# WoodOxen/tactics2d

Hardware: NVIDIA H100
Metric: participant_steps_per_sec (higher is better)
Workload: dtype f32

## Files before the change

tactics2d_b200/csrc/t2d_kernels.cu:

```cuda
#include <cuda_runtime.h>
#include <stdint.h>
#include <stdio.h>
#include <string.h>

#include <algorithm>
#include <atomic>
#include <cmath>
#include <memory>
#include <mutex>
#include <string>
#include <vector>

#include "../../include/t2d_b200.h"
#include "t2d_math.cuh"

namespace t2d {

constexpr int MAX_WARPS_PER_CTA = 8;
constexpr int CTA_THREADS = MAX_WARPS_PER_CTA * 32;
constexpr int PPL = 4;
constexpr int POSE_PER_WARP = 32 * PPL;
constexpr int MAP_SMEM_LIMIT = 120 * 1024;

struct MapHeader {
  int32_t n_seg, gx, gy, n_items;
  float x0, y0, inv_cell, cell;
  uint32_t off_seg, off_cell, off_items, total_bytes;
  uint32_t off_clear;
  int32_t fine;
  uint32_t off_dcell, off_ditems;
  float dil;
  int32_t n_ditems;
  uint32_t off_objfirst;
  int32_t n_poly;
  uint32_t off_poly;
  uint32_t off_pbox;
  uint32_t off_fine;
  uint32_t smem_bytes;
  float bxmin, bxmax, bymin, bymax;
  int32_t has_bounds;
  uint32_t pad[3];
};
constexpr float CLEAR_QUANT = 0.125f;
static_assert(sizeof(MapHeader) == 128, "MapHeader must be 128 bytes");

struct StepArgs {
  float *x, *y, *h, *v, *vx, *vy;
  const uint8_t* type_id;
  int32_t* step_count;
  const float* action;
  const float* ego_action;
  uint8_t* flags;
  int16_t* hit_index;
  int16_t* hit_segment;
  uint8_t* scn_status;
  uint8_t* done;
  const unsigned char* map_blob;
  const uint32_t* tile_off;
  const uint16_t* tile_id;
  MapHeader mh;
  const Params* table;
  int map_bytes, map_in_smem;
  int n_types;
  int N, M, G;
  int g_shift, mp_shift, unused1, n_tiles, wpc, table_bytes;
  int off_poseA, off_poseB, off_hit, off_queue, off_sorted, unused0, off_qcount, off_bar;
  int n_steps;
  float dt, dt_rem;
  double dt_d, dt_rem_d, interval_d;
  int max_step, cfg_flags;
  int do_physics, has_bounds, vec_ok, needs_vel_in;
  int prefetch;
  float bxmin, bxmax, bymin, bymax;
  float rb_max;
  const float* goal_target;
  float* goal_iou;
  float* goal_last_pose;
  int32_t* goal_noact_count;
  float goal_threshold;
  int goal_noact_max;
  float *wheel_f, *wheel_r;
};

__device__ __forceinline__ uint32_t smem_u32(const void* p) { return (uint32_t)__cvta_generic_to_shared(p); }

__device__ __forceinline__ void mbar_init(uint64_t* bar, uint32_t count) {
  asm volatile("mbarrier.init.shared::cta.b64 [%0], %1;" ::"r"(smem_u32(bar)), "r"(count));
}
__device__ __forceinline__ void fence_mbar_init() { asm volatile("fence.mbarrier_init.release.cluster;" ::: "memory"); }
__device__ __forceinline__ void mbar_expect_tx(uint64_t* bar, uint32_t bytes) {
  asm volatile("mbarrier.arrive.expect_tx.shared::cta.b64 _, [%0], %1;" ::"r"(smem_u32(bar)), "r"(bytes) : "memory");
}
__device__ __forceinline__ void bulk_g2s(void* dst, const void* src, uint32_t bytes, uint64_t* bar) {
  asm volatile("cp.async.bulk.shared::cluster.global.mbarrier::complete_tx::bytes [%0], [%1], %2, [%3];" ::"r"(
                   smem_u32(dst)),
               "l"(src), "r"(bytes), "r"(smem_u32(bar))
               : "memory");
}
__device__ __forceinline__ void mbar_wait(uint64_t* bar, uint32_t parity) {
  uint32_t ok = 0;
  while (!ok) {
    asm volatile(
        "{\n\t.reg .pred p;\n\t"
        "mbarrier.try_wait.parity.shared::cta.b64 p, [%1], %2;\n\t"
        "selp.u32 %0, 1, 0, p;\n\t}"
        : "=r"(ok)
        : "r"(smem_u32(bar)), "r"(parity)
        : "memory");
  }
}

template <int BYTES> struct VecOf;
template <> struct VecOf<1> { using T = uint8_t; };
template <> struct VecOf<2> { using T = uint16_t; };
template <> struct VecOf<4> { using T = uint32_t; };
template <> struct VecOf<8> { using T = uint2; };
template <> struct VecOf<16> { using T = uint4; };

template <typename T, int N>
__device__ __forceinline__ void ld_vec(const T* p, T (&o)[N]) {
  using V = typename VecOf<sizeof(T) * N>::T;
  const V v = *reinterpret_cast<const V*>(p);
  memcpy(o, &v, sizeof(V));
}
template <typename T, int N>
__device__ __forceinline__ void st_vec(T* p, const T (&o)[N]) {
  using V = typename VecOf<sizeof(T) * N>::T;
  V v;
  memcpy(&v, o, sizeof(V));
  *reinterpret_cast<V*>(p) = v;
}

struct Pose {
  float x, y, h, c, s, l, w;
};

__device__ __noinline__ bool pair_exact(const Pose a, const Pose b) {
  const bool ca = a.w < 0.0f, cb = b.w < 0.0f;
  if (!ca && !cb) return obb_obb_f64(a.x, a.y, a.h, a.l, a.w, b.x, b.y, b.h, b.l, b.w);
  if (!ca && cb) return obb_circle_f64(a.x, a.y, a.h, a.l, a.w, b.x, b.y, b.l);
  if (ca && !cb) return obb_circle_f64(b.x, b.y, b.h, b.l, b.w, a.x, a.y, a.l);
  return circle_circle_f64(a.x, a.y, a.l, b.x, b.y, b.l);
}

__device__ __forceinline__ bool pair_hit(const Pose& a, const Pose& b) {
  const bool ca = a.w < 0.0f, cb = b.w < 0.0f;
  int r;
  if (!ca && !cb) r = obb_obb_f32(a.x, a.y, a.c, a.s, a.l, a.w, b.x, b.y, b.c, b.s, b.l, b.w);
  else if (!ca && cb) r = obb_circle_f32(a.x, a.y, a.c, a.s, a.l, a.w, b.x, b.y, b.l);
  else if (ca && !cb) r = obb_circle_f32(b.x, b.y, b.c, b.s, b.l, b.w, a.x, a.y, a.l);
  else r = circle_circle_f32(a.x, a.y, a.l, b.x, b.y, b.l);
  if (r < 0) return pair_exact(a, b);
  return r != 0;
}

__device__ __noinline__ bool seg_exact(const Pose a, const float4 sg) {
  if (a.w < 0.0f) return circle_segment_f64(a.x, a.y, a.l, sg.x, sg.y, sg.z, sg.w);
  return obb_segment_f64(a.x, a.y, a.h, a.l, a.w, sg.x, sg.y, sg.z, sg.w);
}

__device__ __forceinline__ bool seg_hit(const Pose& a, const float4 sg) {
  int r = a.w < 0.0f ? circle_segment_f32(a.x, a.y, a.l, sg.x, sg.y, sg.z, sg.w)
                     : obb_segment_f32(a.x, a.y, a.c, a.s, a.l, a.w, sg.x, sg.y, sg.z, sg.w);
  if (r < 0) return seg_exact(a, sg);
  return r != 0;
}

__device__ __noinline__ bool oob_exact(const Pose a, float xmin, float xmax, float ymin, float ymax) {
  return out_of_bound_f64(a.x, a.y, a.h, a.l, a.w, a.w < 0.0f, xmin, xmax, ymin, ymax);
}

__device__ __noinline__ void other_model_step(OneIO& io, const Params& p, int n_steps, double dt, double dt_rem, double interval) {
  if (p.model() == MODEL_DYNAMICS) {
    dynamics_step(io, p, n_steps, dt);
  } else if (p.model() == MODEL_POINTMASS_NEWTON) {
    pointmass_newton_step(io, p, interval);
  } else if (p.model() == MODEL_POINTMASS_EULER) {
    pointmass_euler_step(io, p, n_steps, dt, dt_rem);
  } else {
    sincos_fast(io.h, &io.sh, &io.ch);
  }
}

__device__ __forceinline__ unsigned near_fetch(const float ax, const float ay, const float rbound, const MapHeader& mh, const uint8_t* fine,
                                               unsigned& alt) {
  const float r = rbound * 1.0001f + 1e-3f;
  const float fx = (ax - mh.x0) * mh.inv_cell, fy = (ay - mh.y0) * mh.inv_cell;
  const float gxf = (float)mh.gx, gyf = (float)mh.gy;
  const bool inside = fx >= 0.0f && fy >= 0.0f && fx < gxf && fy < gyf;
  const float kf = (float)mh.fine;
  const int nx = mh.gx * mh.fine, ny = mh.gy * mh.fine;
  const float ux = fmaf(inside ? fx : 0.0f, kf, -0.5f), uy = fmaf(inside ? fy : 0.0f, kf, -0.5f);
  int ix = __float_as_int(ux + RINT_MAGIC) - 0x4B400000, iy = __float_as_int(uy + RINT_MAGIC) - 0x4B400000;
  ix = min(max(ix, 0), nx - 1); iy = min(max(iy, 0), ny - 1);
  const unsigned q = (unsigned)__ldg(fine + (size_t)iy * nx + ix);
  const float ox = fmaxf(fmaxf(-fx, fx - gxf), 0.0f), oy = fmaxf(fmaxf(-fy, fy - gyf), 0.0f);
  const unsigned q_out = fmaxf(ox, oy) * mh.cell <= r ? 0u : 255u;
  alt = inside ? 0xffffffffu : q_out;
  return q;
}
__device__ __forceinline__ bool near_decide(unsigned q, unsigned alt, const float rbound) {
  const unsigned v = alt == 0xffffffffu ? q : alt;
  return (float)v * CLEAR_QUANT <= rbound * 1.0001f + 1e-3f;
}

static_assert(PPL == 4, "pslot's masks and shifts are those of 4 participants per lane");
__device__ __forceinline__ int pslot(int slot) { return ((slot & 3) << 5) | (slot >> 2); }

__device__ __forceinline__ Pose load_pose(const float4* poseA, const float4* poseB, int slot) {
  const int idx = pslot(slot);
  const float4 a = poseA[idx], b = poseB[idx];
  Pose p;
  p.x = a.x; p.y = a.y; p.h = a.w; p.c = b.x; p.s = b.y; p.l = b.z; p.w = b.w;
  return p;
}

constexpr int QCAP = 192;

__device__ __forceinline__ void pair_resolve(int ti, int tj, int mp_shift, const float4* poseA, const float4* poseB, int* hitmin) {
  const Pose a = load_pose(poseA, poseB, ti), b = load_pose(poseA, poseB, tj);
  if (pair_hit(a, b)) {
    const int mask = (1 << mp_shift) - 1;
    atomicMin(&hitmin[pslot(ti)], tj & mask);
    atomicMin(&hitmin[pslot(tj)], ti & mask);
  }
}

__device__ __forceinline__ float neg_reach2(float rb, float rb_max) {
  const float rr = rb + rb_max;
  return -fmaf(rr * rr, 1.00001f, 1e-12f);
}

__device__ __forceinline__ unsigned f2ord(float f) {
  const unsigned u = __float_as_uint(f);
  return (u & 0x80000000u) ? ~u : (u | 0x80000000u);
}
__device__ __forceinline__ float ord2f(unsigned o) { return __uint_as_float((o & 0x80000000u) ? (o & 0x7fffffffu) : ~o); }

__device__ __forceinline__ void sweep_pair(const float4& a, const float4& b, int tb, int M, int Mh, unsigned* queue, int* qcount) {
  const int sa = (int)(__float_as_uint(a.w) & 127u), sb = (int)(__float_as_uint(b.w) & 127u);
  int d = sb - sa;
  if (d < 0) d += M;
  const float dx = b.x - a.x, dy = b.y - a.y;
  if (d <= Mh && fmaf(dx, dx, fmaf(dy, dy, a.z)) <= 0.0f) {
    const int slot = atomicAdd(qcount, 1);
    if (slot < QCAP) queue[slot] = ((unsigned)(tb + sa) << 16) | (unsigned)(tb + sb);
  }
  if (d >= M - Mh && fmaf(dx, dx, fmaf(dy, dy, b.z)) <= 0.0f) {
    const int slot = atomicAdd(qcount, 1);
    if (slot < QCAP) queue[slot] = ((unsigned)(tb + sb) << 16) | (unsigned)(tb + sa);
  }
}

__device__ __forceinline__ float pair_min_margin(const float4& a, const float4& b, float nglob) {
  const float dx = b.x - a.x, dy = b.y - a.y;
  return fmaf(dx, dx, fmaf(dy, dy, nglob));
}

__device__ __noinline__ void pair_exhaustive(int t0, int tb, int m0, int M, int mp_shift, float rb_max, const float4* poseA,
                                             const float4* poseB, int* hitmin) {
  for (int i = 0; i < PPL; ++i) {
    if (m0 + i >= M) break;
    const float4 a = poseA[pslot(t0 + i)];
    if (!(a.x == a.x)) continue;
    const float rr = a.z + rb_max;
    for (int j = m0 + i + 1; j < M; ++j) {
      const float4 b = poseA[pslot(tb + j)];
      const float dx = b.x - a.x, dy = b.y - a.y;
      if (fmaf(dx, dx, dy * dy) <= fmaf(rr * rr, 1.00001f, 1e-12f)) pair_resolve(t0 + i, tb + j, mp_shift, poseA, poseB, hitmin);
    }
  }
}

constexpr int QX0 = 128;

struct MapView {
  const float4* seg;
  const uint32_t* cell_start;
  const uint16_t* items;
  const uint32_t* dcell_start;
  const uint16_t* ditems;
};
__device__ __forceinline__ MapView map_view(const unsigned char* blob, const MapHeader& mh) {
  MapView v;
  v.seg = reinterpret_cast<const float4*>(blob + mh.off_seg);
  v.cell_start = reinterpret_cast<const uint32_t*>(blob + mh.off_cell);
  v.items = reinterpret_cast<const uint16_t*>(blob + mh.off_items);
  v.dcell_start = reinterpret_cast<const uint32_t*>(blob + mh.off_dcell);
  v.ditems = reinterpret_cast<const uint16_t*>(blob + mh.off_ditems);
  return v;
}

__device__ __forceinline__ int static_walk(int ti, const Pose& a, float rbound, const MapHeader& mh, const MapView& mv, unsigned* queue,
                                           int* qcount) {
  const float r = rbound * 1.0001f + 1e-3f;
  if (!(r <= mh.dil)) return -2;
  const float fx = (a.x - mh.x0) * mh.inv_cell, fy = (a.y - mh.y0) * mh.inv_cell;
  if (!(fx >= 0.0f && fy >= 0.0f && fx < (float)mh.gx && fy < (float)mh.gy)) return 0x7fffffff;
  const int cx = min((int)fx, mh.gx - 1), cy = min((int)fy, mh.gy - 1);
  const int cidx = cy * mh.gx + cx;
  const uint32_t b = mv.dcell_start[cidx], e = mv.dcell_start[cidx + 1];
  int best = 0x7fffffff;
  bool overflow = false;
  const float bx0 = a.x - r, bx1 = a.x + r, by0 = a.y - r, by1 = a.y + r;
  for (uint32_t k = b; k < e; ++k) {
    const int sidx = mv.ditems[k];
    const float4 sg = mv.seg[sidx];
    if (fmaxf(sg.x, sg.z) < bx0 || fminf(sg.x, sg.z) > bx1 || fmaxf(sg.y, sg.w) < by0 || fminf(sg.y, sg.w) > by1) continue;
    const int rr = a.w < 0.0f ? circle_segment_f32(a.x, a.y, a.l, sg.x, sg.y, sg.z, sg.w)
                              : obb_segment_f32(a.x, a.y, a.c, a.s, a.l, a.w, sg.x, sg.y, sg.z, sg.w);
    if (rr > 0) {
      best = sidx;
      break;
    } else if (rr < 0) {
      const int slot = atomicAdd(qcount, 1);
      if (slot < QCAP - QX0) queue[QX0 + slot] = ((unsigned)ti << 16) | (unsigned)sidx;
      else overflow = true;
    }
  }
  return overflow ? -2 : best;
}

__device__ __noinline__ int static_objects(int best, float px, float py, const MapHeader& mh, const unsigned char* blob) {
  if (best != 0x7fffffff && best >= 0) best = reinterpret_cast<const uint16_t*>(blob + mh.off_objfirst)[best];
  const int32_t* pstart = reinterpret_cast<const int32_t*>(blob + mh.off_poly);
  const float4* pbox = reinterpret_cast<const float4*>(blob + mh.off_pbox);
  const float4* seg = reinterpret_cast<const float4*>(blob + mh.off_seg);
  for (int p = 0; p < mh.n_poly; ++p) {
    const int s0 = pstart[p];
    if (s0 >= best) break;
    const float4 bb = pbox[p];
    if (!(px >= bb.x && px <= bb.y && py >= bb.z && py <= bb.w)) continue;
    bool in = false;
    for (int i = s0; i < pstart[p + 1]; ++i) {
      const float4 e = seg[i];
      if ((e.y > py) != (e.w > py) && px < (e.z - e.x) * (py - e.y) / (e.w - e.y) + e.x) in = !in;
    }
    if (in) { best = s0; break; }
  }
  return best;
}

__device__ __noinline__ int static_walk_exact(const Pose a, float rbound, const MapHeader mh, const float4* seg, const uint32_t* cell_start,
                                              const uint16_t* items) {
  const float r = rbound * 1.0001f + 1e-3f;
  int cx0 = max((int)floorf((a.x - r - mh.x0) * mh.inv_cell), 0), cx1 = min((int)floorf((a.x + r - mh.x0) * mh.inv_cell), mh.gx - 1);
  int cy0 = max((int)floorf((a.y - r - mh.y0) * mh.inv_cell), 0), cy1 = min((int)floorf((a.y + r - mh.y0) * mh.inv_cell), mh.gy - 1);
  int best = 0x7fffffff;
  for (int cy = cy0; cy <= cy1; ++cy)
    for (int cx = cx0; cx <= cx1; ++cx) {
      const int cidx = cy * mh.gx + cx;
      for (uint32_t k = cell_start[cidx]; k < cell_start[cidx + 1]; ++k) {
        const int sidx = items[k];
        if (sidx >= best) break;
        if (seg_hit(a, seg[sidx])) best = sidx;
      }
    }
  return best;
}

struct TileRef {
  const MapHeader* mh;
  const unsigned char* sec;
  const unsigned char* blob;
};

template <bool MAP_TABLE>
__device__ __forceinline__ void static_phase(unsigned near_bits, int t0, int lane, int tile_first_scn, int mp_shift, const StepArgs& A,
                                             const unsigned char* s_map, const float4* poseA, const float4* poseB, int* segmin,
                                             unsigned* queue, int* qcount) {
  int base = 0;
#pragma unroll
  for (int i = 0; i < PPL; ++i) {
    const bool near = (near_bits >> i) & 1u;
    const unsigned m = __ballot_sync(0xffffffffu, near);
    if (near) queue[base + __popc(m & ((1u << lane) - 1u))] = (unsigned)(t0 + i);
    base += __popc(m);
  }
  auto tile_of = [&](int ti) {
    TileRef t;
    if constexpr (MAP_TABLE) {
      const long long n = (long long)tile_first_scn + (ti >> mp_shift);
      const unsigned char* blob = A.map_blob + A.tile_off[n < A.N ? A.tile_id[n] : 0];
      t.mh = reinterpret_cast<const MapHeader*>(blob); t.sec = blob; t.blob = blob;
    } else {
      t.mh = &A.mh; t.sec = A.map_in_smem ? s_map : A.map_blob; t.blob = A.map_blob;
    }
    return t;
  };
  __syncwarp();
  for (int k = lane; k < base; k += 32) {
    const int ti = (int)queue[k];
    const TileRef t = tile_of(ti);
    const Pose a = load_pose(poseA, poseB, ti);
    const int best = t.mh->n_seg > 0 ? static_walk(ti, a, poseA[pslot(ti)].z, *t.mh, map_view(t.sec, *t.mh), queue, qcount) : 0x7fffffff;
    segmin[pslot(ti)] = best;
  }
  __syncwarp();
  const int n_x = min(*qcount, QCAP - QX0);
  for (int k = lane; k < n_x; k += 32) {
    const unsigned e = queue[QX0 + k];
    const int ti = (int)(e >> 16), sidx = (int)(e & 0xffffu);
    int* sm = &segmin[pslot(ti)];
    if (*sm != -2 && sidx < *sm) {
      const TileRef t = tile_of(ti);
      if (seg_exact(load_pose(poseA, poseB, ti), reinterpret_cast<const float4*>(t.sec + t.mh->off_seg)[sidx])) atomicMin(sm, sidx);
    }
  }
  __syncwarp();
  for (int k = lane; k < base; k += 32) {
    const int ti = (int)queue[k];
    int* sm = &segmin[pslot(ti)];
    const TileRef t = tile_of(ti);
    if (*sm == -2) {
      const MapView mv = map_view(t.sec, *t.mh);
      *sm = static_walk_exact(load_pose(poseA, poseB, ti), poseA[pslot(ti)].z, *t.mh, mv.seg, mv.cell_start, mv.items);
    }
    if (t.mh->n_poly > 0) {
      const float4 pa = poseA[pslot(ti)];
      *sm = static_objects(*sm, pa.x, pa.y, *t.mh, t.blob);
    }
  }
  __syncwarp();
}

__device__ __noinline__ bool oob_slow(const float4* poseA, const float4* poseB, int idx, float xmin, float xmax, float ymin, float ymax) {
  const Pose a = load_pose(poseA, poseB, idx);
  int r = out_of_bound_f32(a.x, a.y, a.c, a.s, a.l, a.w, a.w < 0.0f, xmin, xmax, ymin, ymax);
  if (r < 0) r = out_of_bound_f64(a.x, a.y, a.h, a.l, a.w, a.w < 0.0f, xmin, xmax, ymin, ymax) ? 1 : 0;
  return r != 0;
}

__device__ __noinline__ unsigned ego_goal_events(const StepArgs& A, long long n, float ex, float ey, float eh, float el, float ew) {
  unsigned r = 0;
  float* last = A.goal_last_pose + 4 * n;
  if (A.goal_noact_max > 0) {
    int cnt = A.goal_noact_count[n];
    if (last[3] != 0.0f) {
      const double iou = rect_iou_f64(ex, ey, eh, el, ew, last[0], last[1], last[2], el, ew);
      cnt = iou > 0.999 ? cnt + 1 : 0;
    }
    A.goal_noact_count[n] = cnt;
    if (cnt > A.goal_noact_max) r |= 2u;
  }
  last[0] = ex; last[1] = ey; last[2] = eh; last[3] = 1.0f;
  const float* tg = A.goal_target + 5 * n;
  const double iou = rect_iou_f64(ex, ey, eh, el, ew, tg[0], tg[1], tg[2], tg[3], tg[4]);
  A.goal_iou[n] = (float)iou;
  if (iou >= (double)A.goal_threshold) r |= 1u;
  return r;
}

__device__ __forceinline__ void prefetch_tile_l2(const StepArgs& A, long long i) {
  asm volatile("prefetch.global.L2 [%0];" ::"l"(A.x + i));
  asm volatile("prefetch.global.L2 [%0];" ::"l"(A.y + i));
  asm volatile("prefetch.global.L2 [%0];" ::"l"(A.h + i));
  asm volatile("prefetch.global.L2 [%0];" ::"l"(A.v + i));
  if (A.action) asm volatile("prefetch.global.L2 [%0];" ::"l"(A.action + 2 * i));
  asm volatile("prefetch.global.L2 [%0];" ::"l"(A.type_id + i));
  if (A.needs_vel_in) {
    asm volatile("prefetch.global.L2 [%0];" ::"l"(A.vx + i));
    asm volatile("prefetch.global.L2 [%0];" ::"l"(A.vy + i));
  }
}

template <bool KIN_ONLY, bool MAP_TABLE>
__global__ void __launch_bounds__(CTA_THREADS, 2) t2d_step_kernel(const __grid_constant__ StepArgs A) {
  extern __shared__ __align__(128) unsigned char smem[];
  const int map_smem_bytes = (!MAP_TABLE && A.map_in_smem) ? A.map_bytes : 0;
  const int table_bytes = A.table_bytes;
  const int wpc = A.wpc;
  unsigned char* s_map = smem;
  Params* s_table = reinterpret_cast<Params*>(smem + map_smem_bytes);
  float4* s_poseA = reinterpret_cast<float4*>(smem + A.off_poseA);
  float4* s_poseB = reinterpret_cast<float4*>(smem + A.off_poseB);
  int* s_hit = reinterpret_cast<int*>(smem + A.off_hit);
  unsigned* s_queue = reinterpret_cast<unsigned*>(smem + A.off_queue);
  float4* s_sorted = reinterpret_cast<float4*>(smem + A.off_sorted);
  int* s_qcount = reinterpret_cast<int*>(smem + A.off_qcount);
  uint64_t* s_bar = reinterpret_cast<uint64_t*>(smem + A.off_bar);

  const int tid = threadIdx.x, lane = tid & 31, warp = tid >> 5;
  asm volatile("griddepcontrol.launch_dependents;" ::: "memory");

  if (tid == 0) {
    mbar_init(s_bar, 1);
    fence_mbar_init();
  }
  __syncthreads();
  if (tid == 0) {
    mbar_expect_tx(s_bar, (uint32_t)(table_bytes + map_smem_bytes));
    bulk_g2s(s_table, A.table, (uint32_t)table_bytes, s_bar);
    if (map_smem_bytes > 0) bulk_g2s(s_map, A.map_blob, (uint32_t)map_smem_bytes, s_bar);
  }
  bool staged = false;
  {
    const long long n_ = ((long long)blockIdx.x * wpc + warp) * (32 >> A.g_shift) + (lane >> A.g_shift);
    const int m_ = (lane & (A.G - 1)) * PPL;
    if (A.prefetch && n_ < A.N && m_ < A.M) prefetch_tile_l2(A, n_ * A.M + m_);
  }
  asm volatile("griddepcontrol.wait;" ::: "memory");
  const int G = A.G, M = A.M;
  const int spw = 32 >> A.g_shift;
  const int sub = lane >> A.g_shift;
  const int gl = lane & (G - 1);
  const int m0 = gl * PPL;
  const int MP = G * PPL;
  float4* poseA = s_poseA + warp * POSE_PER_WARP;
  float4* poseB = s_poseB + warp * POSE_PER_WARP;
  int* hitmin = s_hit + warp * POSE_PER_WARP;
  unsigned* queue = s_queue + warp * QCAP;
  int* qcount = s_qcount + warp;
  const int tb = sub * MP, t0 = tb + m0;
  const int mp_shift = A.mp_shift;
  float4* sorted = s_sorted + warp * POSE_PER_WARP + tb;
  const int Mh = M >> 1;

  const int n_tiles = A.n_tiles;
  for (int tile = (int)blockIdx.x * wpc + warp; tile < n_tiles; tile += (int)gridDim.x * wpc) {
    const long long n = (long long)tile * spw + sub;
    const bool scn_ok = n < A.N;
    int nvalid = scn_ok ? min(PPL, M - m0) : 0;
    if (nvalid < 0) nvalid = 0;
    const long long idx0 = n * M + m0;

    float sx[PPL], sy[PPL], shd[PPL], sv[PPL], svx[PPL], svy[PPL], a0[PPL], a1[PPL];
    int tidv[PPL];
#pragma unroll
    for (int i = 0; i < PPL; ++i) {
      sx[i] = sy[i] = shd[i] = sv[i] = svx[i] = svy[i] = a0[i] = a1[i] = 0.0f;
      tidv[i] = T2D_TYPE_INACTIVE;
    }
    if (nvalid == PPL && A.vec_ok) {
      ld_vec<float, PPL>(A.x + idx0, sx);
      ld_vec<float, PPL>(A.y + idx0, sy);
      ld_vec<float, PPL>(A.h + idx0, shd);
      ld_vec<float, PPL>(A.v + idx0, sv);
      uint8_t tb8[PPL];
      ld_vec<uint8_t, PPL>(A.type_id + idx0, tb8);
#pragma unroll
      for (int i = 0; i < PPL; ++i) tidv[i] = tb8[i];
      if (A.do_physics) {
        float2 act[PPL];
        float lo[4], hi[4];
        ld_vec<float, 4>(A.action + 2 * idx0, lo);
        ld_vec<float, 4>(A.action + 2 * idx0 + 4, hi);
        act[0] = make_float2(lo[0], lo[1]); act[1] = make_float2(lo[2], lo[3]);
        act[2] = make_float2(hi[0], hi[1]); act[3] = make_float2(hi[2], hi[3]);
#pragma unroll
        for (int i = 0; i < PPL; ++i) { a0[i] = act[i].x; a1[i] = act[i].y; }
        if (A.needs_vel_in) {
          ld_vec<float, PPL>(A.vx + idx0, svx);
          ld_vec<float, PPL>(A.vy + idx0, svy);
        }
      }
    } else {
#pragma unroll
      for (int i = 0; i < PPL; ++i) {
        if (i < nvalid) {
          sx[i] = A.x[idx0 + i]; sy[i] = A.y[idx0 + i]; shd[i] = A.h[idx0 + i]; sv[i] = A.v[idx0 + i];
          tidv[i] = A.type_id[idx0 + i];
          if (A.do_physics) {
            a0[i] = A.action[2 * (idx0 + i)]; a1[i] = A.action[2 * (idx0 + i) + 1];
            if (A.needs_vel_in) { svx[i] = A.vx[idx0 + i]; svy[i] = A.vy[idx0 + i]; }
          }
        }
      }
    }
    {
      const long long n_next = n + (long long)gridDim.x * wpc * spw;
      if (A.prefetch && n_next < A.N && m0 < M) prefetch_tile_l2(A, n_next * M + m0);
    }
    if (A.ego_action != nullptr && A.do_physics && gl == 0 && scn_ok) {
      const float2 ea = reinterpret_cast<const float2*>(A.ego_action)[n];
      a0[0] = ea.x; a1[0] = ea.y;
    }
    if (!staged) {
      mbar_wait(s_bar, 0);
      staged = true;
    }
    float ch[PPL], sh[PPL];
    bool active[PPL], kin[PPL];
    const Params* pp[PPL];
    int model[PPL];
    bool lane_all_kin = true, lane_any_kin = false;
#pragma unroll
    for (int i = 0; i < PPL; ++i) {
      active[i] = tidv[i] < A.n_types;
      pp[i] = &s_table[active[i] ? tidv[i] : 0];
      model[i] = pp[i]->model_shape & 0xff;
      kin[i] = active[i] && (model[i] == MODEL_KINEMATICS);
      lane_all_kin = lane_all_kin && kin[i];
      lane_any_kin = lane_any_kin || kin[i];
      ch[i] = 1.0f; sh[i] = 0.0f;
    }
    if (A.cfg_flags & T2D_CFG_STEER_FIRST) {
#pragma unroll
      for (int i = 0; i < PPL; ++i)
        if (model[i] <= MODEL_DYNAMICS || model[i] == MODEL_DRIFT) { float t = a0[i]; a0[i] = a1[i]; a1[i] = t; }
    }

    if (A.do_physics) {
      if (__any_sync(0xffffffffu, lane_any_kin)) {
        const Params* const null_row = &s_table[A.n_types];
        const Params* pk[PPL];
        KinIO<PPL> io;
#pragma unroll
        for (int i = 0; i < PPL; ++i) {
          pk[i] = kin[i] ? pp[i] : null_row;
          io.x[i] = kin[i] ? sx[i] : 0.0f; io.y[i] = kin[i] ? sy[i] : 0.0f;
          io.h[i] = kin[i] ? shd[i] : 0.0f; io.v[i] = kin[i] ? sv[i] : 0.0f;
          io.acc[i] = kin[i] ? a0[i] : 0.0f; io.steer[i] = kin[i] ? a1[i] : 0.0f;
        }
        kinematics_step<PPL>(io, pk, A.n_steps, A.dt, A.dt_rem);
#pragma unroll
        for (int i = 0; i < PPL; ++i) {
          if (kin[i]) {
            sx[i] = io.x[i]; sy[i] = io.y[i]; shd[i] = io.h[i]; sv[i] = io.v[i];
            svx[i] = io.vx[i]; svy[i] = io.vy[i]; ch[i] = io.ch[i]; sh[i] = io.sh[i];
          }
        }
      }
      if (!lane_all_kin) {
#pragma unroll
        for (int i = 0; i < PPL; ++i) {
          if (active[i] && !kin[i]) {
            if constexpr (!KIN_ONLY) {
              OneIO io;
              io.x = sx[i]; io.y = sy[i]; io.h = shd[i]; io.v = sv[i]; io.vx = svx[i]; io.vy = svy[i];
              io.a0 = a0[i]; io.a1 = a1[i];
              io.ch = 1.0f; io.sh = 0.0f;
              other_model_step(io, *pp[i], A.n_steps, A.dt_d, A.dt_rem_d, A.interval_d);
              sx[i] = io.x; sy[i] = io.y; shd[i] = io.h; sv[i] = io.v; svx[i] = io.vx; svy[i] = io.vy;
              ch[i] = io.ch; sh[i] = io.sh;
            } else {
              sincos_fast(shd[i], &sh[i], &ch[i]);
            }
          }
        }
      }
      bool all_active = true;
#pragma unroll
      for (int i = 0; i < PPL; ++i) all_active = all_active && active[i];
      if (nvalid == PPL && A.vec_ok && all_active) {
        st_vec<float, PPL>(A.x + idx0, sx);
        st_vec<float, PPL>(A.y + idx0, sy);
        st_vec<float, PPL>(A.h + idx0, shd);
        st_vec<float, PPL>(A.v + idx0, sv);
        st_vec<float, PPL>(A.vx + idx0, svx);
        st_vec<float, PPL>(A.vy + idx0, svy);
      } else {
#pragma unroll
        for (int i = 0; i < PPL; ++i) {
          if (i < nvalid && active[i]) {
            A.x[idx0 + i] = sx[i]; A.y[idx0 + i] = sy[i]; A.h[idx0 + i] = shd[i]; A.v[idx0 + i] = sv[i];
            A.vx[idx0 + i] = svx[i]; A.vy[idx0 + i] = svy[i];
          }
        }
      }
    } else {
#pragma unroll
      for (int i = 0; i < PPL; ++i) sincos_fast(shd[i], &sh[i], &ch[i]);
    }

    float px[PPL], py[PPL], rb[PPL];
    unsigned solid_bits = 0;
#pragma unroll
    for (int i = 0; i < PPL; ++i) {
      const Vec4 g2 = params_group(pp[i], 2);
      const bool sol = active[i] && (__float_as_int(g2.w) >> 8) != SHAPE_NONE;
      solid_bits |= sol ? (1u << i) : 0u;
      rb[i] = g2.z;
      px[i] = sol ? sx[i] : __int_as_float(0x7fc00000);
      py[i] = sy[i];
      poseA[i * 32 + lane] = make_float4(px[i], py[i], rb[i], shd[i]);
      poseB[i * 32 + lane] = make_float4(ch[i], sh[i], g2.x, g2.y);
    }
    if (lane == 0) *qcount = 0;
    __syncwarp();
    const int cnt_in = (A.do_physics && gl == 0 && scn_ok) ? A.step_count[n] : 0;

    unsigned near_q[PPL], near_alt[PPL];
#pragma unroll
    for (int i = 0; i < PPL; ++i) { near_q[i] = 255u; near_alt[i] = 255u; }
    const MapHeader* lane_mh = &A.mh;
    const unsigned char* lane_blob = A.map_blob;
    if constexpr (MAP_TABLE) {
      lane_blob = A.map_blob + A.tile_off[scn_ok ? A.tile_id[n] : 0];
      lane_mh = reinterpret_cast<const MapHeader*>(lane_blob);
    }
    if (A.map_blob != nullptr && lane_mh->n_seg > 0) {
#pragma unroll
      for (int i = 0; i < PPL; ++i) {
        unsigned alt;
        near_q[i] = near_fetch(px[i], py[i], rb[i], *lane_mh, lane_blob + lane_mh->off_fine, alt);
        near_alt[i] = ((solid_bits >> i) & 1u) ? alt : 255u;
      }
    }

    int hit[PPL];
    {
      unsigned key[PPL];
#pragma unroll
      for (int i = 0; i < PPL; ++i)
        key[i] = (px[i] == px[i] ? (f2ord(px[i]) & ~127u) : 0xffffff80u) | (unsigned)(m0 + i);
      auto cx = [&](int a, int b, bool desc) {
        const unsigned lo = min(key[a], key[b]), hi = max(key[a], key[b]);
        key[a] = desc ? hi : lo;
        key[b] = desc ? lo : hi;
      };
      cx(0, 1, false); cx(2, 3, true);
      for (int S = PPL; S <= MP; S <<= 1) {
        const bool desc = (gl & (S >> 2)) != 0;
        for (int j = S >> 3; j > 0; j >>= 1) {
          const bool keep_max = ((gl & j) != 0) != desc;
#pragma unroll
          for (int i = 0; i < PPL; ++i) {
            const unsigned o = __shfl_xor_sync(0xffffffffu, key[i], j);
            key[i] = keep_max ? max(key[i], o) : min(key[i], o);
          }
        }
        cx(0, 2, desc); cx(1, 3, desc); cx(0, 1, desc); cx(2, 3, desc);
      }
      float4 own[PPL];
#pragma unroll
      for (int i = 0; i < PPL; ++i) {
// ... 2454 lines not shown
```

Baseline: 14.42 billion.

## Load-balance static segment walk across warp lanes via prefix-sum work distribution

Replaces the per-lane static_walk loop, where each lane walked its own pose's cell segment list, with a warp-cooperative scheme. A shuffle-based prefix sum over per-pose list lengths and a binary search let each lane test one (pose, segment) pair, so lanes stay busy when list lengths differ. Hits are merged with atomicMin instead of an early break, and the exact-fallback and polygon pass is skipped when no lane flagged a rare case. It gives up the early exit per pose and adds shuffles and atomics. It also relies on segmin being initialised elsewhere and on the minimum segment index matching the old first-hit result.

```diff
diff --git a/tactics2d_b200/csrc/t2d_kernels.cu b/tactics2d_b200/csrc/t2d_kernels.cu
--- a/tactics2d_b200/csrc/t2d_kernels.cu
+++ b/tactics2d_b200/csrc/t2d_kernels.cu
@@ -291,36 +291,6 @@
   return v;
 }
 
-__device__ __forceinline__ int static_walk(int ti, const Pose& a, float rbound, const MapHeader& mh, const MapView& mv, unsigned* queue,
-                                           int* qcount) {
-  const float r = rbound * 1.0001f + 1e-3f;
-  if (!(r <= mh.dil)) return -2;
-  const float fx = (a.x - mh.x0) * mh.inv_cell, fy = (a.y - mh.y0) * mh.inv_cell;
-  if (!(fx >= 0.0f && fy >= 0.0f && fx < (float)mh.gx && fy < (float)mh.gy)) return 0x7fffffff;
-  const int cx = min((int)fx, mh.gx - 1), cy = min((int)fy, mh.gy - 1);
-  const int cidx = cy * mh.gx + cx;
-  const uint32_t b = mv.dcell_start[cidx], e = mv.dcell_start[cidx + 1];
-  int best = 0x7fffffff;
-  bool overflow = false;
-  const float bx0 = a.x - r, bx1 = a.x + r, by0 = a.y - r, by1 = a.y + r;
-  for (uint32_t k = b; k < e; ++k) {
-    const int sidx = mv.ditems[k];
-    const float4 sg = mv.seg[sidx];
-    if (fmaxf(sg.x, sg.z) < bx0 || fminf(sg.x, sg.z) > bx1 || fmaxf(sg.y, sg.w) < by0 || fminf(sg.y, sg.w) > by1) continue;
-    const int rr = a.w < 0.0f ? circle_segment_f32(a.x, a.y, a.l, sg.x, sg.y, sg.z, sg.w)
-                              : obb_segment_f32(a.x, a.y, a.c, a.s, a.l, a.w, sg.x, sg.y, sg.z, sg.w);
-    if (rr > 0) {
-      best = sidx;
-      break;
-    } else if (rr < 0) {
-      const int slot = atomicAdd(qcount, 1);
-      if (slot < QCAP - QX0) queue[QX0 + slot] = ((unsigned)ti << 16) | (unsigned)sidx;
-      else overflow = true;
-    }
-  }
-  return overflow ? -2 : best;
-}
-
 __device__ __noinline__ int static_objects(int best, float px, float py, const MapHeader& mh, const unsigned char* blob) {
   if (best != 0x7fffffff && best >= 0) best = reinterpret_cast<const uint16_t*>(blob + mh.off_objfirst)[best];
   const int32_t* pstart = reinterpret_cast<const int32_t*>(blob + mh.off_poly);
@@ -389,39 +359,100 @@
     return t;
   };
   __syncwarp();
-  for (int k = lane; k < base; k += 32) {
-    const int ti = (int)queue[k];
-    const TileRef t = tile_of(ti);
-    const Pose a = load_pose(poseA, poseB, ti);
-    const int best = t.mh->n_seg > 0 ? static_walk(ti, a, poseA[pslot(ti)].z, *t.mh, map_view(t.sec, *t.mh), queue, qcount) : 0x7fffffff;
-    segmin[pslot(ti)] = best;
+  bool rare = false;
+  for (int c0 = 0; c0 < base; c0 += 32) {
+    int ti = 0, len = 0, kb = 0;
+    if (c0 + lane < base) {
+      ti = (int)queue[c0 + lane];
+      const TileRef t = tile_of(ti);
+      rare |= t.mh->n_poly > 0;
+      if (t.mh->n_seg > 0) {
+        const float4 pa = poseA[pslot(ti)];
+        const float r = pa.z * 1.0001f + 1e-3f;
+        const float fx = (pa.x - t.mh->x0) * t.mh->inv_cell, fy = (pa.y - t.mh->y0) * t.mh->inv_cell;
+        if (!(r <= t.mh->dil)) {
+          segmin[pslot(ti)] = -2;
+          rare = true;
+        } else if (fx >= 0.0f && fy >= 0.0f && fx < (float)t.mh->gx && fy < (float)t.mh->gy) {
+          const int cx = min((int)fx, t.mh->gx - 1), cy = min((int)fy, t.mh->gy - 1);
+          const uint32_t* dcs = map_view(t.sec, *t.mh).dcell_start + cy * t.mh->gx + cx;
+          kb = (int)dcs[0];
+          len = (int)dcs[1] - kb;
+        }
+      }
+    }
+    int off = len;
+#pragma unroll
+    for (int o = 1; o < 32; o <<= 1)
+      asm("{\n\t.reg .s32 v;\n\t.reg .pred p;\n\tshfl.sync.up.b32 v|p, %0, %1, 0, 0xffffffff;\n\t@p add.s32 %0, %0, v;\n\t}"
+          : "+r"(off) : "r"(o));
+    const int total = __shfl_sync(0xffffffffu, off, 31);
+    off -= len;
+    kb -= off;
+    for (int p0 = 0; p0 < total; p0 += 32) {
+      const int j = p0 + lane;
+      int L = 0;
+#pragma unroll
+      for (int s = 16; s > 0; s >>= 1)
+        if (__shfl_sync(0xffffffffu, off, L + s) <= j) L += s;
+      const int pti = __shfl_sync(0xffffffffu, ti, L);
+      const int k = __shfl_sync(0xffffffffu, kb, L) + j;
+      if (j < total) {
+        const TileRef t = tile_of(pti);
+        const MapView mv = map_view(t.sec, *t.mh);
+        const float4 pa = poseA[pslot(pti)], pb = poseB[pslot(pti)];
+        const float r = pa.z * 1.0001f + 1e-3f;
+        const int sidx = mv.ditems[k];
+        const float4 sg = mv.seg[sidx];
+        if (!(fmaxf(sg.x, sg.z) < pa.x - r || fminf(sg.x, sg.z) > pa.x + r || fmaxf(sg.y, sg.w) < pa.y - r ||
+              fminf(sg.y, sg.w) > pa.y + r)) {
+          const int rr = pb.w < 0.0f ? circle_segment_f32(pa.x, pa.y, pb.z, sg.x, sg.y, sg.z, sg.w)
+                                     : obb_segment_f32(pa.x, pa.y, pb.x, pb.y, pb.z, pb.w, sg.x, sg.y, sg.z, sg.w);
+          if (rr > 0) {
+            atomicMin(&segmin[pslot(pti)], sidx);
+          } else if (rr < 0) {
+            const int slot = atomicAdd(qcount, 1);
+            if (slot < QCAP - QX0) {
+              queue[QX0 + slot] = ((unsigned)pti << 16) | (unsigned)sidx;
+            } else {
+              atomicMin(&segmin[pslot(pti)], -2);
+              rare = true;
+            }
+          }
+        }
+      }
+    }
   }
   __syncwarp();
   const int n_x = min(*qcount, QCAP - QX0);
-  for (int k = lane; k < n_x; k += 32) {
-    const unsigned e = queue[QX0 + k];
-    const int ti = (int)(e >> 16), sidx = (int)(e & 0xffffu);
-    int* sm = &segmin[pslot(ti)];
-    if (*sm != -2 && sidx < *sm) {
+  if (n_x > 0) {
+    for (int k = lane; k < n_x; k += 32) {
+      const unsigned e = queue[QX0 + k];
+      const int ti = (int)(e >> 16), sidx = (int)(e & 0xffffu);
+      int* sm = &segmin[pslot(ti)];
+      if (*sm != -2 && sidx < *sm) {
+        const TileRef t = tile_of(ti);
+        if (seg_exact(load_pose(poseA, poseB, ti), reinterpret_cast<const float4*>(t.sec + t.mh->off_seg)[sidx])) atomicMin(sm, sidx);
+      }
+    }
+    __syncwarp();
+  }
+  if (__any_sync(0xffffffffu, rare)) {
+    for (int k = lane; k < base; k += 32) {
+      const int ti = (int)queue[k];
+      int* sm = &segmin[pslot(ti)];
       const TileRef t = tile_of(ti);
-      if (seg_exact(load_pose(poseA, poseB, ti), reinterpret_cast<const float4*>(t.sec + t.mh->off_seg)[sidx])) atomicMin(sm, sidx);
-    }
-  }
-  __syncwarp();
-  for (int k = lane; k < base; k += 32) {
-    const int ti = (int)queue[k];
-    int* sm = &segmin[pslot(ti)];
-    const TileRef t = tile_of(ti);
-    if (*sm == -2) {
-      const MapView mv = map_view(t.sec, *t.mh);
-      *sm = static_walk_exact(load_pose(poseA, poseB, ti), poseA[pslot(ti)].z, *t.mh, mv.seg, mv.cell_start, mv.items);
-    }
-    if (t.mh->n_poly > 0) {
-      const float4 pa = poseA[pslot(ti)];
-      *sm = static_objects(*sm, pa.x, pa.y, *t.mh, t.blob);
-    }
-  }
-  __syncwarp();
+      if (*sm == -2) {
+        const MapView mv = map_view(t.sec, *t.mh);
+        *sm = static_walk_exact(load_pose(poseA, poseB, ti), poseA[pslot(ti)].z, *t.mh, mv.seg, mv.cell_start, mv.items);
+      }
+      if (t.mh->n_poly > 0) {
+        const float4 pa = poseA[pslot(ti)];
+        *sm = static_objects(*sm, pa.x, pa.y, *t.mh, t.blob);
+      }
+    }
+    __syncwarp();
+  }
 }
 
 __device__ __noinline__ bool oob_slow(const float4* poseA, const float4* poseB, int idx, float xmin, float xmax, float ymin, float ymax) {
```

New measurement: 14.38 billion (median of 6 runs). No clear change (-0.3%).
